# crisbodnar/text-to-image

Measured on AMD Instinct MI355X. Metric: images/sec (G+D step) at 64x64 batch=64, higher is better.
Workload: dtype f32; 1 GPU; wgancls 64x64 batch=64/GPU fp32, synthetic images + random 1024-d text embeddings, D step (+kt) then G step, Adam(b1=0,b2=0.9); global_batch=64, parallelism=dp1, launch=hipGraph replay (1 graph/iteration)

## Files before the change

### text-to-image_amd/csrc/t2i_thin.hip

```cpp
#include <hip/hip_runtime.h>
#include <stdint.h>

#include "t2i_internal.h"

namespace t2i {

template <int CI, bool DYH = false>
__global__ __launch_bounds__(256) void thin_deconv_k4s2_kernel(const void* __restrict__ dyv, const float* __restrict__ w,
                                                               const float* __restrict__ bias, float* __restrict__ dx,
                                                               int H, int W, int Co, int CH, int act, float alpha) {
  extern __shared__ __attribute__((aligned(16))) float tile[];
  const int Ho = H >> 1, Wo = W >> 1;
  const int PS = CH + 4;
  const int b = blockIdx.z;
  const int ih0 = blockIdx.y * 16, iw0 = blockIdx.x * 16;
  const int oh0 = (ih0 >> 1) - 1, ow0 = (iw0 >> 1) - 1;
  const int c4n = CH >> 2;
  float* wlds = tile + 100 * PS;
  const int wv = __builtin_amdgcn_readfirstlane(threadIdx.x >> 6);
  const int ph = wv >> 1, pw = wv & 1;
  const int lane = threadIdx.x & 63;
  const int py = lane >> 3, px = lane & 7;
  const int kh0 = (ph + 1) & 1, kw0 = (pw + 1) & 1;
  float acc[CI];
#pragma unroll
  for (int ci = 0; ci < CI; ++ci) acc[ci] = 0.f;
  for (int cbase = 0; cbase < Co; cbase += CH) {
    if (cbase) __syncthreads();
    if (CH == 64) {
      constexpr int C4N = 16, XN = (100 * C4N + 255) / 256, WN = (16 * CI * C4N + 255) / 256;
      float4 xv[XN], wv[WN];
#pragma unroll
      for (int u = 0; u < XN; ++u) {
        const int i = threadIdx.x + 256 * u;
        const int pix = i >> 4, c4 = i & 15;
        const int r = pix / 10, c = pix - r * 10;
        const int oh = oh0 + r, ow = ow0 + c;
        float4 v = make_float4(0.f, 0.f, 0.f, 0.f);
        if (i < 100 * C4N && (unsigned)oh < (unsigned)Ho && (unsigned)ow < (unsigned)Wo) {
          const size_t e = ((size_t)(b * Ho + oh) * Wo + ow) * Co + cbase + c4 * 4;
          if (DYH) {
            const uint2 q = *reinterpret_cast<const uint2*>(reinterpret_cast<const unsigned short*>(dyv) + e);
            v = make_float4(__uint_as_float(q.x << 16), __uint_as_float(q.x & 0xFFFF0000u), __uint_as_float(q.y << 16), __uint_as_float(q.y & 0xFFFF0000u));
          } else {
            v = *reinterpret_cast<const float4*>(reinterpret_cast<const float*>(dyv) + e);
          }
        }
        xv[u] = v;
      }
#pragma unroll
      for (int u = 0; u < WN; ++u) {
        const int i = threadIdx.x + 256 * u;
        const int row = i >> 4, c4 = i & 15;
        wv[u] = i < 16 * CI * C4N ? *reinterpret_cast<const float4*>(w + (size_t)row * Co + cbase + c4 * 4) : make_float4(0.f, 0.f, 0.f, 0.f);
      }
#pragma unroll
      for (int u = 0; u < XN; ++u) {
        const int i = threadIdx.x + 256 * u;
        if (i < 100 * C4N) *reinterpret_cast<float4*>(&tile[(i >> 4) * PS + (i & 15) * 4]) = xv[u];
      }
#pragma unroll
      for (int u = 0; u < WN; ++u) {
        const int i = threadIdx.x + 256 * u;
        if (i < 16 * CI * C4N) reinterpret_cast<float4*>(wlds)[i] = wv[u];
      }
    } else {
    for (int i = threadIdx.x; i < 100 * c4n; i += 256) {
      const int pix = i / c4n, c4 = i - pix * c4n;
      const int r = pix / 10, c = pix - r * 10;
      const int oh = oh0 + r, ow = ow0 + c;
      float4 v = make_float4(0.f, 0.f, 0.f, 0.f);
      if ((unsigned)oh < (unsigned)Ho && (unsigned)ow < (unsigned)Wo) {
        const size_t e = ((size_t)(b * Ho + oh) * Wo + ow) * Co + cbase + c4 * 4;
        if (DYH) {
          const uint2 u = *reinterpret_cast<const uint2*>(reinterpret_cast<const unsigned short*>(dyv) + e);
          v = make_float4(__uint_as_float(u.x << 16), __uint_as_float(u.x & 0xFFFF0000u), __uint_as_float(u.y << 16), __uint_as_float(u.y & 0xFFFF0000u));
        } else {
          v = *reinterpret_cast<const float4*>(reinterpret_cast<const float*>(dyv) + e);
        }
      }
      *reinterpret_cast<float4*>(&tile[pix * PS + c4 * 4]) = v;
    }
    for (int i = threadIdx.x; i < 16 * CI * c4n; i += 256) {
      const int row = i / c4n, c4 = i - row * c4n;
      reinterpret_cast<float4*>(wlds)[i] = *reinterpret_cast<const float4*>(w + (size_t)row * Co + cbase + c4 * 4);
    }
    }
    __syncthreads();
#pragma unroll
    for (int jh = 0; jh < 2; ++jh) {
#pragma unroll
      for (int jw = 0; jw < 2; ++jw) {
        const int r = py + 1 + ph - jh, c = px + 1 + pw - jw;
        const float* src = &tile[(r * 10 + c) * PS];
        const float* wt = wlds + (((kh0 + 2 * jh) * 4 + (kw0 + 2 * jw)) * CI) * CH;
#pragma unroll 4
        for (int c4 = 0; c4 < c4n; ++c4) {
          const float4 d = *reinterpret_cast<const float4*>(src + c4 * 4);
#pragma unroll
          for (int ci = 0; ci < CI; ++ci) {
            const float4 f = *reinterpret_cast<const float4*>(wt + ci * CH + c4 * 4);
            acc[ci] = fmaf(d.x, f.x, fmaf(d.y, f.y, fmaf(d.z, f.z, fmaf(d.w, f.w, acc[ci]))));
          }
        }
      }
    }
  }
  const int ih = ih0 + 2 * py + ph, iw = iw0 + 2 * px + pw;
  float* o = dx + ((size_t)(b * H + ih) * W + iw) * CI;
#pragma unroll
  for (int ci = 0; ci < CI; ++ci) o[ci] = apply_act(acc[ci] + (bias ? bias[ci] : 0.f), act, alpha);
}

bool thin_deconv_eligible(const t2i_conv_desc& d) {
  return d.KH == 4 && d.KW == 4 && d.SH == 2 && d.SW == 2 && d.pad_t == 1 && d.pad_l == 1 && d.Cin >= 1 && d.Cin <= 4 &&
         (d.Cout % 4) == 0 && d.Cout >= 16 && d.Cout <= 512 && (d.H % 16) == 0 && (d.W % 16) == 0 && d.Ho * 2 == d.H &&
         d.Wo * 2 == d.W;
}

hipError_t thin_deconv_launch(const t2i_conv_desc& d, const void* dy, const float* w, const float* bias, float* dx,
                              int act, float alpha, hipStream_t stream, bool dy_bf16) {
  int parts = tuning().thin_parts;
  if (parts < 1) parts = 1;
  while (parts > 1 && ((d.Cout % (4 * parts)) != 0 || d.Cout / parts < 32)) parts >>= 1;
  const int CH = d.Cout / parts;
  const size_t lds = ((size_t)100 * (CH + 4) + (size_t)16 * d.Cin * CH) * sizeof(float);
  dim3 grid(d.W / 16, d.H / 16, d.B);
#define T2I_THIN(CI)                                                                                              \
  case CI: {                                                                                                      \
    auto k = dy_bf16 ? thin_deconv_k4s2_kernel<CI, true> : thin_deconv_k4s2_kernel<CI, false>;                    \
    if (lds > 48 * 1024) {                                                                                        \
      hipError_t e = hipFuncSetAttribute(reinterpret_cast<const void*>(k), hipFuncAttributeMaxDynamicSharedMemorySize, (int)lds); \
      if (e != hipSuccess) return e;                                                                              \
    }                                                                                                             \
    hipLaunchKernelGGL(k, grid, dim3(256), lds, stream, dy, w, bias, dx, d.H, d.W, d.Cout, CH, act, alpha);       \
    break;                                                                                                        \
  }
  switch (d.Cin) {
    T2I_THIN(1) T2I_THIN(2) T2I_THIN(3) T2I_THIN(4)
    default: return hipErrorInvalidValue;
  }
#undef T2I_THIN
  return hipGetLastError();
}

template <bool BWD>
__global__ __launch_bounds__(256) void tiny_conv_kernel(const float* __restrict__ in, const float* __restrict__ w,
                                                        const float* __restrict__ bias, float* __restrict__ out,
                                                        t2i_conv_desc d, int act, float alpha) {
  const int OH = BWD ? d.H : d.Ho, OW = BWD ? d.W : d.Wo, OC = BWD ? d.Cin : d.Cout;
  const int IH = BWD ? d.Ho : d.H, IW = BWD ? d.Wo : d.W, IC = BWD ? d.Cout : d.Cin;
  const size_t npix = (size_t)d.B * OH * OW;
  for (size_t p = (size_t)blockIdx.x * blockDim.x + threadIdx.x; p < npix; p += (size_t)gridDim.x * blockDim.x) {
    const int ow = (int)(p % OW);
    const size_t t = p / OW;
    const int oh = (int)(t % OH);
    const int b = (int)(t / OH);
    float acc[4] = {0.f, 0.f, 0.f, 0.f};
    for (int kh = 0; kh < d.KH; ++kh) {
      const int ih = BWD ? oh + d.pad_t - kh : oh * d.SH - d.pad_t + kh;
      if ((unsigned)ih >= (unsigned)IH) continue;
      for (int kw = 0; kw < d.KW; ++kw) {
        const int iw = BWD ? ow + d.pad_l - kw : ow * d.SW - d.pad_l + kw;
        if ((unsigned)iw >= (unsigned)IW) continue;
        const float* src = in + ((size_t)(b * IH + ih) * IW + iw) * IC;
        const float* wt = w + (size_t)(kh * d.KW + kw) * d.Cin * d.Cout;
        for (int ic = 0; ic < IC; ++ic) {
          const float v = src[ic];
#pragma unroll
          for (int oc = 0; oc < 4; ++oc)
            if (oc < OC) acc[oc] = fmaf(v, BWD ? wt[oc * d.Cout + ic] : wt[ic * d.Cout + oc], acc[oc]);
        }
      }
    }
    float* o = out + p * OC;
#pragma unroll
    for (int oc = 0; oc < 4; ++oc)
      if (oc < OC) o[oc] = apply_act(acc[oc] + (bias ? bias[oc] : 0.f), act, alpha);
  }
}

bool tiny_conv_eligible(const t2i_conv_desc& d, bool bwd) {
  if (d.Cin > 4 || d.Cout > 4) return false;
  if (bwd && (d.SH != 1 || d.SW != 1)) return false;
  return true;
}

hipError_t tiny_conv_launch(const t2i_conv_desc& d, bool bwd, const float* in, const float* w, const float* bias,
                            float* out, int act, float alpha, hipStream_t stream) {
  const size_t npix = (size_t)d.B * (bwd ? d.H * d.W : d.Ho * d.Wo);
  size_t blocks = (npix + 255) / 256;
  if (blocks > 4096) blocks = 4096;
  if (blocks < 1) blocks = 1;
  if (bwd)
    hipLaunchKernelGGL(tiny_conv_kernel<true>, dim3((unsigned)blocks), dim3(256), 0, stream, in, w, bias, out, d, act, alpha);
  else
    hipLaunchKernelGGL(tiny_conv_kernel<false>, dim3((unsigned)blocks), dim3(256), 0, stream, in, w, bias, out, d, act, alpha);
  return hipGetLastError();
}

}

namespace t2i {

__global__ __launch_bounds__(256) void head_fwd_kernel(const float* __restrict__ x, const float* __restrict__ w,
                                                       const float* __restrict__ bias, float* __restrict__ y, int K,
                                                       int Co, int act, float alpha) {
  __shared__ float red[4][4];
  const float* row = x + (size_t)blockIdx.x * K;
  float acc[4] = {0.f, 0.f, 0.f, 0.f};
  if (Co == 1 && (K & 3) == 0 && ((reinterpret_cast<uintptr_t>(x) | reinterpret_cast<uintptr_t>(w)) & 15) == 0) {
    float4 a4 = make_float4(0.f, 0.f, 0.f, 0.f);
#pragma unroll 4
    for (int j = threadIdx.x; j < (K >> 2); j += 256) {
      const float4 v = reinterpret_cast<const float4*>(row)[j];
      const float4 q = reinterpret_cast<const float4*>(w)[j];
      a4.x = fmaf(v.x, q.x, a4.x); a4.y = fmaf(v.y, q.y, a4.y); a4.z = fmaf(v.z, q.z, a4.z); a4.w = fmaf(v.w, q.w, a4.w);
    }
    acc[0] = (a4.x + a4.y) + (a4.z + a4.w);
  } else
  for (int j = threadIdx.x; j < K; j += 256) {
    const float v = row[j];
#pragma unroll
    for (int co = 0; co < 4; ++co)
      if (co < Co) acc[co] = fmaf(v, w[(size_t)j * Co + co], acc[co]);
  }
#pragma unroll
  for (int co = 0; co < 4; ++co) {
#pragma unroll
    for (int o = 32; o > 0; o >>= 1) acc[co] += __shfl_xor(acc[co], o, 64);
    if ((threadIdx.x & 63) == 0) red[threadIdx.x >> 6][co] = acc[co];
  }
  __syncthreads();
  if (threadIdx.x < Co) {
    const int co = threadIdx.x;
    const float s = (red[0][co] + red[1][co]) + (red[2][co] + red[3][co]) + (bias ? bias[co] : 0.f);
    y[(size_t)blockIdx.x * Co + co] = apply_act(s, act, alpha);
  }
}

__global__ __launch_bounds__(256) void head_bwd_data_kernel(const float* __restrict__ dy, const float* __restrict__ w,
                                                            float* __restrict__ dx, int B, int K, int Co) {
  const size_t n = (size_t)B * K;
  for (size_t i = (size_t)blockIdx.x * blockDim.x + threadIdx.x; i < n; i += (size_t)gridDim.x * blockDim.x) {
    const size_t b = i / K;
    const int j = (int)(i - b * K);
    float s = 0.f;
    for (int co = 0; co < Co; ++co) s = fmaf(dy[b * Co + co], w[(size_t)j * Co + co], s);
    dx[i] = s;
  }
}

__global__ __launch_bounds__(256) void head_bwd_filter_kernel(const float* __restrict__ x, const float* __restrict__ dy,
                                                              float* __restrict__ dw, int B, int K, int Co, int accumulate) {
  __shared__ float red[4][64][4];
  const int tx = threadIdx.x & 63, ty = threadIdx.x >> 6;
  const int j = blockIdx.x * 64 + tx;
  float acc[4] = {0.f, 0.f, 0.f, 0.f};
  if (j < K) {
    for (int b = ty; b < B; b += 4) {
      const float v = x[(size_t)b * K + j];
#pragma unroll
      for (int co = 0; co < 4; ++co)
        if (co < Co) acc[co] = fmaf(v, dy[b * Co + co], acc[co]);
    }
  }
#pragma unroll
  for (int co = 0; co < 4; ++co) red[ty][tx][co] = acc[co];
  __syncthreads();
  if (ty == 0 && j < K) {
#pragma unroll
    for (int co = 0; co < 4; ++co)
      if (co < Co) {
        const float s = (red[0][tx][co] + red[1][tx][co]) + (red[2][tx][co] + red[3][tx][co]);
        float* o = dw + (size_t)j * Co + co;
        *o = accumulate ? *o + s : s;
      }
  }
}

bool head_conv_eligible(const t2i_conv_desc& d) {
  return d.Ho == 1 && d.Wo == 1 && d.KH == d.H && d.KW == d.W && d.pad_t == 0 && d.pad_l == 0 && d.Cout <= 4;
}

hipError_t head_fwd_launch(const t2i_conv_desc& d, const float* x, const float* w, const float* bias, float* y, int act,
                           float alpha, hipStream_t stream) {
  hipLaunchKernelGGL(head_fwd_kernel, dim3(d.B), dim3(256), 0, stream, x, w, bias, y, d.H * d.W * d.Cin, d.Cout, act, alpha);
  return hipGetLastError();
}

hipError_t head_bwd_data_launch(const t2i_conv_desc& d, const float* dy, const float* w, float* dx, hipStream_t stream) {
  const int K = d.H * d.W * d.Cin;
  size_t blocks = ((size_t)d.B * K + 255) / 256;
  if (blocks > 4096) blocks = 4096;
  hipLaunchKernelGGL(head_bwd_data_kernel, dim3((unsigned)blocks), dim3(256), 0, stream, dy, w, dx, d.B, K, d.Cout);
  return hipGetLastError();
}

hipError_t head_bwd_filter_launch(const t2i_conv_desc& d, const float* x, const float* dy, float* dw, int accumulate,
                                  hipStream_t stream) {
  const int K = d.H * d.W * d.Cin;
  hipLaunchKernelGGL(head_bwd_filter_kernel, dim3((K + 63) / 64), dim3(256), 0, stream, x, dy, dw, d.B, K, d.Cout, accumulate);
  return hipGetLastError();
}

}

namespace t2i {

typedef float f32x16_t __attribute__((ext_vector_type(16)));

template <int CI, int NB>
__global__ __launch_bounds__(256) void stem_k4s2_fwd_kernel(const float* __restrict__ x, const float* __restrict__ w,
                                                            const float* __restrict__ bias, float* __restrict__ y, int H, int W,
                                                            int act, float alpha, __bf16* __restrict__ yh) {
  constexpr int K = 16 * CI, Co = 32 * NB;
  extern __shared__ __attribute__((aligned(16))) float lds_stem[];
  const int Wo = W >> 1, Ho = H >> 1;
  constexpr int cols = 66 * CI;
  float* xs = lds_stem;
  float* ws = lds_stem + 10 * cols;
  const int b = blockIdx.z, oh0 = blockIdx.y * 4, ow0 = blockIdx.x * 32;
  constexpr int XN = (10 * cols + 255) / 256, WN = (K * Co / 4 + 255) / 256;
  float xv[XN];
  float4 wv[WN];
#pragma unroll
  for (int u = 0; u < XN; ++u) {
    const int i = threadIdx.x + 256 * u;
    const int r = i / cols, j = i - r * cols;
    const int px = j / CI, ci = j - px * CI;
    const int ih = 2 * oh0 - 1 + r, iw = 2 * ow0 - 1 + px;
    const bool ok = i < 10 * cols && (unsigned)ih < (unsigned)H && (unsigned)iw < (unsigned)W;
    xv[u] = ok ? x[((size_t)(b * H + ih) * W + iw) * CI + ci] : 0.f;
  }
#pragma unroll
  for (int u = 0; u < WN; ++u) {
    const int i = threadIdx.x + 256 * u;
    wv[u] = i < K * Co / 4 ? reinterpret_cast<const float4*>(w)[i] : make_float4(0.f, 0.f, 0.f, 0.f);
  }
#pragma unroll
  for (int u = 0; u < XN; ++u) {
    const int i = threadIdx.x + 256 * u;
    if (i < 10 * cols) xs[i] = xv[u];
  }
#pragma unroll
  for (int u = 0; u < WN; ++u) {
    const int i = threadIdx.x + 256 * u;
    if (i < K * Co / 4) reinterpret_cast<float4*>(ws)[i] = wv[u];
  }
  __syncthreads();
  const int lane = threadIdx.x & 63, wave = threadIdx.x >> 6;
  const int l31 = lane & 31, lh = lane >> 5;
  f32x16_t acc[NB];
#pragma unroll
  for (int j = 0; j < NB; ++j)
#pragma unroll
    for (int e = 0; e < 16; ++e) acc[j][e] = 0.f;
#pragma unroll
  for (int s2 = 0; s2 < K / 2; ++s2) {
    const int k = 2 * s2 + lh;
    const int tap = k / CI, ci = k - tap * CI;
    const int kh = tap >> 2, kw = tap & 3;
    const float a = xs[(2 * wave + kh) * cols + (2 * l31 + kw) * CI + ci];
#pragma unroll
    for (int j = 0; j < NB; ++j)
      acc[j] = __builtin_amdgcn_mfma_f32_32x32x2f32(a, ws[k * Co + j * 32 + l31], acc[j], 0, 0, 0);
  }
  const int oh = oh0 + wave;
  if constexpr (NB % 2 == 0) {
    constexpr int SROW = 68;
    __syncthreads();
    float* st = lds_stem + wave * (32 * SROW);
#pragma unroll
    for (int half = 0; half < NB / 2; ++half) {
#pragma unroll
      for (int jj = 0; jj < 2; ++jj)
#pragma unroll
        for (int e = 0; e < 16; ++e) st[((e & 3) + 8 * (e >> 2) + 4 * lh) * SROW + jj * 32 + l31] = acc[half * 2 + jj][e];
      __builtin_amdgcn_fence(__ATOMIC_RELEASE, "wavefront");
      __builtin_amdgcn_wave_barrier();
      __builtin_amdgcn_fence(__ATOMIC_ACQUIRE, "wavefront");
#pragma unroll
      for (int it = 0; it < 4; ++it) {
        const int idx = it * 64 + lane, row = idx >> 3, c8 = idx & 7;
        const float4 v0 = *reinterpret_cast<const float4*>(&st[row * SROW + c8 * 8]);
        const float4 v1 = *reinterpret_cast<const float4*>(&st[row * SROW + c8 * 8 + 4]);
        const int ow = ow0 + row, ch = half * 64 + c8 * 8;
        if (oh < Ho && ow < Wo) {
          float v[8] = {v0.x, v0.y, v0.z, v0.w, v1.x, v1.y, v1.z, v1.w};
          if (bias) {
            const float4 b0 = *reinterpret_cast<const float4*>(bias + ch), b1 = *reinterpret_cast<const float4*>(bias + ch + 4);
            v[0] += b0.x; v[1] += b0.y; v[2] += b0.z; v[3] += b0.w; v[4] += b1.x; v[5] += b1.y; v[6] += b1.z; v[7] += b1.w;
          } else {
#pragma unroll
            for (int k = 0; k < 8; ++k) v[k] += 0.f;
          }
#pragma unroll
          for (int k = 0; k < 8; ++k) v[k] = apply_act(v[k], act, alpha);
          const size_t o = ((size_t)(b * Ho + oh) * Wo + ow) * Co + ch;
          if (y) {
            *reinterpret_cast<float4*>(y + o) = make_float4(v[0], v[1], v[2], v[3]);
            *reinterpret_cast<float4*>(y + o + 4) = make_float4(v[4], v[5], v[6], v[7]);
          }
          if (yh) {
            typedef float f2_t __attribute__((ext_vector_type(2)));
            typedef __bf16 h2_t __attribute__((ext_vector_type(2)));
            uint4 h;
            { f2_t t = {v[0], v[1]}; h.x = __builtin_bit_cast(unsigned, __builtin_convertvector(t, h2_t)); }
            { f2_t t = {v[2], v[3]}; h.y = __builtin_bit_cast(unsigned, __builtin_convertvector(t, h2_t)); }
            { f2_t t = {v[4], v[5]}; h.z = __builtin_bit_cast(unsigned, __builtin_convertvector(t, h2_t)); }
            { f2_t t = {v[6], v[7]}; h.w = __builtin_bit_cast(unsigned, __builtin_convertvector(t, h2_t)); }
            *reinterpret_cast<uint4*>(reinterpret_cast<unsigned short*>(yh) + o) = h;
          }
        }
      }
      __builtin_amdgcn_fence(__ATOMIC_RELEASE, "wavefront");
      __builtin_amdgcn_wave_barrier();
      __builtin_amdgcn_fence(__ATOMIC_ACQUIRE, "wavefront");
    }
  } else if (oh < Ho) {
#pragma unroll
    for (int j = 0; j < NB; ++j) {
      const float bv = bias ? bias[j * 32 + l31] : 0.f;
#pragma unroll
      for (int e = 0; e < 16; ++e) {
        const int ow = ow0 + (e & 3) + 8 * (e >> 2) + 4 * lh;
        if (ow < Wo) {
          const float v = apply_act(acc[j][e] + bv, act, alpha);
          const size_t o = ((size_t)(b * Ho + oh) * Wo + ow) * Co + j * 32 + l31;
          if (y) y[o] = v;
          if (yh) yh[o] = (__bf16)v;
        }
      }
    }
  }
}

bool stem_fwd_eligible(const t2i_conv_desc& d) {
  return d.KH == 4 && d.KW == 4 && d.SH == 2 && d.SW == 2 && d.pad_t == 1 && d.pad_l == 1 && d.Cin == 3 && (d.Cout == 128 || d.Cout == 64) &&
         (d.H & 1) == 0 && (d.W & 1) == 0 && d.Ho * 2 == d.H && d.Wo * 2 == d.W;
}

hipError_t stem_fwd_launch(const t2i_conv_desc& d, const float* x, const float* w, const float* bias, float* y, int act, float alpha,
                           hipStream_t stream, void* y_h) {
  size_t lds = ((size_t)10 * 66 * 3 + (size_t)48 * d.Cout) * sizeof(float);
  if (lds < (size_t)4 * 32 * 68 * sizeof(float)) lds = (size_t)4 * 32 * 68 * sizeof(float);
  auto k = d.Cout == 128 ? stem_k4s2_fwd_kernel<3, 4> : stem_k4s2_fwd_kernel<3, 2>;
  dim3 grid((d.Wo + 31) / 32, (d.Ho + 3) / 4, d.B);
  hipLaunchKernelGGL(k, grid, dim3(256), lds, stream, x, w, bias, y, d.H, d.W, act, alpha, reinterpret_cast<__bf16*>(y_h));
  return hipGetLastError();
}

}

namespace t2i {

size_t col_reduce_ws(int64_t rows, int C);
hipError_t col_reduce_launch(const void*, const void*, const float*, int64_t, int, float*, float*, int, void*, hipStream_t, bool in_bf16 = false);

template <int CI, int CO>
__global__ __launch_bounds__(256) void tiny_bwdw_kernel(const float* __restrict__ x, const float* __restrict__ dy,
                                                        float* __restrict__ part, t2i_conv_desc d) {
  __shared__ float red[4][9 * CI * CO];
  float acc[9][CI][CO];
#pragma unroll
  for (int t = 0; t < 9; ++t)
#pragma unroll
    for (int ci = 0; ci < CI; ++ci)
#pragma unroll
      for (int co = 0; co < CO; ++co) acc[t][ci][co] = 0.f;
  const size_t npix = (size_t)d.B * d.Ho * d.Wo;
  for (size_t p = (size_t)blockIdx.x * blockDim.x + threadIdx.x; p < npix; p += (size_t)gridDim.x * blockDim.x) {
    const int ow = (int)(p % d.Wo);
    const size_t t = p / d.Wo;
    const int oh = (int)(t % d.Ho), b = (int)(t / d.Ho);
    float g[CO];
#pragma unroll
    for (int co = 0; co < CO; ++co) g[co] = dy[p * CO + co];
#pragma unroll
    for (int kh = 0; kh < 3; ++kh) {
      const int ih = oh * d.SH - d.pad_t + kh;
#pragma unroll
      for (int kw = 0; kw < 3; ++kw) {
        const int iw = ow * d.SW - d.pad_l + kw;
        if (kh < d.KH && kw < d.KW && (unsigned)ih < (unsigned)d.H && (unsigned)iw < (unsigned)d.W) {
          const float* s = x + ((size_t)(b * d.H + ih) * d.W + iw) * CI;
#pragma unroll
          for (int ci = 0; ci < CI; ++ci) {
            const float v = s[ci];
#pragma unroll
            for (int co = 0; co < CO; ++co) acc[kh * 3 + kw][ci][co] = fmaf(v, g[co], acc[kh * 3 + kw][ci][co]);
          }
        }
      }
    }
  }
#pragma unroll
  for (int t = 0; t < 9; ++t)
#pragma unroll
    for (int ci = 0; ci < CI; ++ci)
#pragma unroll
      for (int co = 0; co < CO; ++co) {
        float v = acc[t][ci][co];
#pragma unroll
        for (int o = 32; o > 0; o >>= 1) v += __shfl_xor(v, o, 64);
        if ((threadIdx.x & 63) == 0) red[threadIdx.x >> 6][(t * CI + ci) * CO + co] = v;
      }
  __syncthreads();
  if (threadIdx.x < 9 * CI * CO) {
    const int i = threadIdx.x;
    const int t = i / (CI * CO), r = i - t * (CI * CO);
    const int kh = t / 3, kw = t - kh * 3;
    if (kh < d.KH && kw < d.KW)
      part[(size_t)blockIdx.x * (d.KH * d.KW * CI * CO) + (kh * d.KW + kw) * (CI * CO) + r] =
          (red[0][i] + red[1][i]) + (red[2][i] + red[3][i]);
  }
}

typedef float stem_f32x16 __attribute__((ext_vector_type(16)));

template <bool DYH, int NB = 4>
__global__ __launch_bounds__(256) void stem_k4s2_bwdf_kernel(const float* __restrict__ x, const void* __restrict__ dy, float* __restrict__ part,
                                                             int B, int H, int W, int Ho, int Wo, int pix_per_wave, FastDiv div_wo, FastDiv div_ho) {
  extern __shared__ __attribute__((aligned(16))) float red[];
  constexpr int CO = 32 * NB;
  const int tid = threadIdx.x, lane = tid & 63, wave = tid >> 6;
  const int l31 = lane & 31, lh = lane >> 5;
  const int P = B * Ho * Wo;
  const int p_begin = (blockIdx.x * 4 + wave) * pix_per_wave;
  int p_end = p_begin + pix_per_wave;
  if (p_end > P) p_end = P;
  int a_off[2]; bool a_ok[2]; int a_kh[2], a_kw[2];
#pragma unroll
  for (int blk = 0; blk < 2; ++blk) {
    const int m = blk * 32 + l31;
    a_ok[blk] = m < 48;
    const int tap = m / 3, ci = m - tap * 3;
    a_kh[blk] = tap >> 2; a_kw[blk] = tap & 3;
    a_off[blk] = (a_kh[blk] * W + a_kw[blk]) * 3 + ci;
  }
  stem_f32x16 acc[2][NB];
#pragma unroll
  for (int i = 0; i < 2; ++i)
#pragma unroll
    for (int j = 0; j < NB; ++j)
#pragma unroll
      for (int e = 0; e < 16; ++e) acc[i][j][e] = 0.f;

  const __amdgpu_buffer_rsrc_t rx = __builtin_amdgcn_make_buffer_rsrc(const_cast<float*>(x), (short)0, (int)((size_t)B * H * W * 3 * 4), 0x00020000);
  const __amdgpu_buffer_rsrc_t ry = __builtin_amdgcn_make_buffer_rsrc(const_cast<void*>(dy), (short)0, (int)((size_t)P * CO * (DYH ? 2 : 4)), 0x00020000);
  constexpr unsigned OOB = 0xFFFFFFF0u;
  auto load = [&](int p, float (&a)[2], float (&b)[NB]) __attribute__((always_inline)) {
    const int pix = p + lh;
    const bool ok = pix < p_end;
    const int pp = ok ? pix : p_begin;
    const int t = div_wo.div(pp);
    const int ow = pp - t * Wo;
    const int img = div_ho.div(t);
    const int oh = t - img * Ho;
    const int ih0 = 2 * oh - 1, iw0 = 2 * ow - 1;
    const int xbase = ((img * H + ih0) * W + iw0) * 3;
#pragma unroll
    for (int blk = 0; blk < 2; ++blk) {
      const bool in = ok & a_ok[blk] & ((unsigned)(ih0 + a_kh[blk]) < (unsigned)H) & ((unsigned)(iw0 + a_kw[blk]) < (unsigned)W);
      a[blk] = __builtin_bit_cast(float, __builtin_amdgcn_raw_buffer_load_b32(rx, in ? (unsigned)(xbase + a_off[blk]) * 4u : OOB, 0, 0));
    }
    constexpr unsigned ES = DYH ? 2u : 4u;
    const unsigned ybase = ok ? ((unsigned)pp * (unsigned)CO + (unsigned)l31) * ES : OOB;
#pragma unroll
    for (int j = 0; j < NB; ++j) {
      if (DYH) b[j] = __uint_as_float((unsigned)(unsigned short)__builtin_amdgcn_raw_buffer_load_b16(ry, ok ? ybase + j * 32u * ES : OOB, 0, 0) << 16);
      else b[j] = __builtin_bit_cast(float, __builtin_amdgcn_raw_buffer_load_b32(ry, ok ? ybase + j * 32u * ES : OOB, 0, 0));
    }
  };

  float a0[4][2], b0[4][NB], a1[4][2], b1[4][NB];
  auto load8 = [&](int p, float (&a)[4][2], float (&b)[4][NB]) __attribute__((always_inline)) {
#pragma unroll
    for (int s = 0; s < 4; ++s) load(p + 2 * s, a[s], b[s]);
  };
  auto mma8 = [&](float (&a)[4][2], float (&b)[4][NB]) __attribute__((always_inline)) {
#pragma unroll
    for (int s = 0; s < 4; ++s)
#pragma unroll
      for (int i = 0; i < 2; ++i)
#pragma unroll
        for (int j = 0; j < NB; ++j) acc[i][j] = __builtin_amdgcn_mfma_f32_32x32x2f32(a[s][i], b[s][j], acc[i][j], 0, 0, 0);
  };
  load8(p_begin, a0, b0);
  for (int p = p_begin; p < p_end; p += 16) {
    load8(p + 8, a1, b1);
    mma8(a0, b0);
    load8(p + 16, a0, b0);
    mma8(a1, b1);
  }

  auto put = [&](float* buf) __attribute__((always_inline)) {
#pragma unroll
    for (int i = 0; i < 2; ++i)
#pragma unroll
      for (int j = 0; j < NB; ++j)
#pragma unroll
        for (int e = 0; e < 16; ++e) buf[(i * 32 + (e & 3) + 8 * (e >> 2) + 4 * lh) * CO + j * 32 + l31] = acc[i][j][e];
  };
  auto add = [&](const float* buf) __attribute__((always_inline)) {
#pragma unroll
    for (int i = 0; i < 2; ++i)
#pragma unroll
      for (int j = 0; j < NB; ++j)
#pragma unroll
        for (int e = 0; e < 16; ++e) acc[i][j][e] += buf[(i * 32 + (e & 3) + 8 * (e >> 2) + 4 * lh) * CO + j * 32 + l31];
  };
  float* buf0 = red;
  float* buf1 = red + 64 * CO;
  if (wave == 2) put(buf0);
  if (wave == 3) put(buf1);
  __syncthreads();
  if (wave == 0) add(buf0);
  if (wave == 1) add(buf1);
  __syncthreads();
  if (wave == 1) put(buf0);
  __syncthreads();
  if (wave == 0) {
    add(buf0);
    float* o = part + (size_t)blockIdx.x * 48 * CO;
#pragma unroll
    for (int i = 0; i < 2; ++i)
#pragma unroll
      for (int j = 0; j < NB; ++j)
#pragma unroll
        for (int e = 0; e < 16; ++e) {
          const int m = i * 32 + (e & 3) + 8 * (e >> 2) + 4 * lh;
          if (m < 48) o[m * CO + j * 32 + l31] = acc[i][j][e];
        }
  }
}

bool stem_bwdf_eligible(const t2i_conv_desc& d) { return stem_fwd_eligible(d); }

static int stem_bwdf_groups(const t2i_conv_desc& d, int* pix_per_wave) {
  const long P = (long)d.B * d.Ho * d.Wo;
  long ppw = (P + 1023) / 1024;
  if (ppw < 16) ppw = 16;
  ppw = (ppw + 15) & ~15L;
  *pix_per_wave = (int)ppw;
  return (int)((P + 4 * ppw - 1) / (4 * ppw));
}

size_t stem_bwdf_ws(const t2i_conv_desc& d) {
  int ppw;
  return (size_t)stem_bwdf_groups(d, &ppw) * 48 * d.Cout * sizeof(float);
}

hipError_t stem_bwdf_launch(const t2i_conv_desc& d, const float* x, const void* dy, float* dw, int accumulate, void* ws, hipStream_t stream, bool dy_bf16) {
  int ppw;
  const int G = stem_bwdf_groups(d, &ppw);
  float* part = reinterpret_cast<float*>(ws);
  const size_t lds = (size_t)2 * 64 * d.Cout * sizeof(float);
  auto k = d.Cout == 128 ? (dy_bf16 ? stem_k4s2_bwdf_kernel<true, 4> : stem_k4s2_bwdf_kernel<false, 4>)
                         : (dy_bf16 ? stem_k4s2_bwdf_kernel<true, 2> : stem_k4s2_bwdf_kernel<false, 2>);
  hipError_t e = hipFuncSetAttribute(reinterpret_cast<const void*>(k), hipFuncAttributeMaxDynamicSharedMemorySize, (int)lds);
  if (e != hipSuccess) return e;
  FastDiv dwo, dho;
  dwo.set((uint32_t)d.Wo); dho.set((uint32_t)d.Ho);
  hipLaunchKernelGGL(k, dim3(G), dim3(256), lds, stream, x, dy, part, d.B, d.H, d.W, d.Ho, d.Wo, ppw, dwo, dho);
  e = hipGetLastError();
  if (e != hipSuccess) return e;
  return splitk_reduce_launch(part, G, (size_t)48 * d.Cout, nullptr, d.Cout, T2I_ACT_NONE, 0.f, dw, accumulate, stream);
}

bool tiny_bwdw_eligible(const t2i_conv_desc& d) { return d.Cin == 3 && d.Cout == 3 && d.KH <= 3 && d.KW <= 3; }

static int tiny_bwdw_blocks(const t2i_conv_desc& d) {
  size_t npix = (size_t)d.B * d.Ho * d.Wo;
  size_t blocks = (npix + 256 * 8 - 1) / (256 * 8);
  if (blocks > 512) blocks = 512;
  if (blocks < 1) blocks = 1;
  return (int)blocks;
}

size_t tiny_bwdw_ws(const t2i_conv_desc& d) {
  const int nb = tiny_bwdw_blocks(d), C = d.KH * d.KW * 9;
  return (size_t)nb * C * sizeof(float) + col_reduce_ws(nb, C) + 256;
}

hipError_t tiny_bwdw_launch(const t2i_conv_desc& d, const float* x, const float* dy, float* dw, int accumulate, void* ws,
                            hipStream_t stream) {
  const int nb = tiny_bwdw_blocks(d), C = d.KH * d.KW * 9;
  float* part = reinterpret_cast<float*>(ws);
  char* ws2 = reinterpret_cast<char*>(ws) + (((size_t)nb * C * sizeof(float) + 255) & ~(size_t)255);
  hipLaunchKernelGGL((tiny_bwdw_kernel<3, 3>), dim3(nb), dim3(256), 0, stream, x, dy, part, d);
  return col_reduce_launch(part, nullptr, nullptr, nb, C, dw, nullptr, accumulate, ws2, stream);
}

}
```

Before: 5085 images/sec.

## Add specialized 3x3 3-channel conv kernels and vectorized head filter gradient

```diff
diff --git a/text-to-image_amd/csrc/t2i_thin.hip b/text-to-image_amd/csrc/t2i_thin.hip
--- a/text-to-image_amd/csrc/t2i_thin.hip
+++ b/text-to-image_amd/csrc/t2i_thin.hip
@@ -180,6 +180,98 @@
   }
 }
 
+template <bool V4>
+__device__ __forceinline__ void load_px6(const float* __restrict__ in, int q0, int npix, float (&v)[18]) {
+  const float* s = in + (ptrdiff_t)q0 * 3;
+  if (V4) {
+    const bool l = (unsigned)q0 < (unsigned)npix, m = (unsigned)(q0 + 1) < (unsigned)npix, r = (unsigned)(q0 + 5) < (unsigned)npix;
+    const float4 z = make_float4(0.f, 0.f, 0.f, 0.f);
+    const float4 a = m ? *reinterpret_cast<const float4*>(s + 3) : z, b = m ? *reinterpret_cast<const float4*>(s + 7) : z,
+                 c = m ? *reinterpret_cast<const float4*>(s + 11) : z;
+#pragma unroll
+    for (int e = 0; e < 3; ++e) { v[e] = l ? s[e] : 0.f; v[15 + e] = r ? s[15 + e] : 0.f; }
+    v[3] = a.x; v[4] = a.y; v[5] = a.z; v[6] = a.w; v[7] = b.x; v[8] = b.y; v[9] = b.z; v[10] = b.w;
+    v[11] = c.x; v[12] = c.y; v[13] = c.z; v[14] = c.w;
+  } else {
+#pragma unroll
+    for (int t = 0; t < 6; ++t) {
+      const bool ok = (unsigned)(q0 + t) < (unsigned)npix;
+#pragma unroll
+      for (int e = 0; e < 3; ++e) v[3 * t + e] = ok ? s[3 * t + e] : 0.f;
+    }
+  }
+}
+
+template <bool V4>
+__device__ __forceinline__ void load_nbhd4(const float* __restrict__ in, int p0, int npix, int H, int W, float (&m)[4][3][3][3]) {
+  float v[3][18];
+#pragma unroll
+  for (int r = 0; r < 3; ++r) load_px6<V4>(in, p0 - 1 + (r - 1) * W, npix, v[r]);
+  int w = p0 % W, h = (p0 / W) % H;
+#pragma unroll
+  for (int j = 0; j < 4; ++j) {
+#pragma unroll
+    for (int r = 0; r < 3; ++r)
+#pragma unroll
+      for (int c = 0; c < 3; ++c) {
+        const bool ok = (unsigned)(h + r - 1) < (unsigned)H && (unsigned)(w + c - 1) < (unsigned)W;
+#pragma unroll
+        for (int ch = 0; ch < 3; ++ch) m[j][r][c][ch] = ok ? v[r][3 * (j + c) + ch] : 0.f;
+      }
+    if (++w == W) { w = 0; if (++h == H) h = 0; }
+  }
+}
+
+template <bool BWD, bool V4>
+__global__ __launch_bounds__(256) void tiny_conv3_kernel(const float* __restrict__ in, const float* __restrict__ w,
+                                                         const float* __restrict__ bias, float* __restrict__ out, int H, int W,
+                                                         int npix, int act, float alpha) {
+  const int quads = (npix + 3) >> 2;
+  for (int q = blockIdx.x * 256 + threadIdx.x; q < quads; q += gridDim.x * 256) {
+    const int p0 = q * 4;
+    float m[4][3][3][3];
+    load_nbhd4<V4>(in, p0, npix, H, W, m);
+    float acc[4][3];
+#pragma unroll
+    for (int j = 0; j < 4; ++j)
+#pragma unroll
+      for (int oc = 0; oc < 3; ++oc) acc[j][oc] = 0.f;
+#pragma unroll
+    for (int kh = 0; kh < 3; ++kh)
+#pragma unroll
+      for (int kw = 0; kw < 3; ++kw)
+#pragma unroll
+        for (int ic = 0; ic < 3; ++ic)
+#pragma unroll
+          for (int oc = 0; oc < 3; ++oc) {
+            const float f = w[(kh * 3 + kw) * 9 + (BWD ? oc * 3 + ic : ic * 3 + oc)];
+#pragma unroll
+            for (int j = 0; j < 4; ++j) acc[j][oc] = fmaf(BWD ? m[j][2 - kh][2 - kw][ic] : m[j][kh][kw][ic], f, acc[j][oc]);
+          }
+    float o[12];
+#pragma unroll
+    for (int j = 0; j < 4; ++j)
+#pragma unroll
+      for (int oc = 0; oc < 3; ++oc) o[3 * j + oc] = apply_act(acc[j][oc] + (bias ? bias[oc] : 0.f), act, alpha);
+    float* dst = out + (size_t)p0 * 3;
+    if (V4) {
+      reinterpret_cast<float4*>(dst)[0] = make_float4(o[0], o[1], o[2], o[3]);
+      reinterpret_cast<float4*>(dst)[1] = make_float4(o[4], o[5], o[6], o[7]);
+      reinterpret_cast<float4*>(dst)[2] = make_float4(o[8], o[9], o[10], o[11]);
+    } else {
+#pragma unroll
+      for (int e = 0; e < 12; ++e)
+        if (p0 + e / 3 < npix) dst[e] = o[e];
+    }
+  }
+}
+
+static bool conv3_k3s1_same(const t2i_conv_desc& d) {
+  return d.Cin == 3 && d.Cout == 3 && d.KH == 3 && d.KW == 3 && d.SH == 1 && d.SW == 1 && d.pad_t == 1 && d.pad_l == 1 && d.Ho == d.H &&
+         d.Wo == d.W && (size_t)d.B * d.H * d.W < ((size_t)1 << 30);
+}
+static bool ptr16(const void* p) { return (reinterpret_cast<uintptr_t>(p) & 15) == 0; }
+
 bool tiny_conv_eligible(const t2i_conv_desc& d, bool bwd) {
   if (d.Cin > 4 || d.Cout > 4) return false;
   if (bwd && (d.SH != 1 || d.SW != 1)) return false;
@@ -189,6 +281,15 @@
 hipError_t tiny_conv_launch(const t2i_conv_desc& d, bool bwd, const float* in, const float* w, const float* bias,
                             float* out, int act, float alpha, hipStream_t stream) {
   const size_t npix = (size_t)d.B * (bwd ? d.H * d.W : d.Ho * d.Wo);
+  if (conv3_k3s1_same(d)) {
+    size_t qb = ((npix + 3) / 4 + 255) / 256;
+    if (qb > 4096) qb = 4096;
+    const bool v4 = (d.W & 3) == 0 && ptr16(in) && ptr16(out);
+    auto k = bwd ? (v4 ? tiny_conv3_kernel<true, true> : tiny_conv3_kernel<true, false>)
+                 : (v4 ? tiny_conv3_kernel<false, true> : tiny_conv3_kernel<false, false>);
+    hipLaunchKernelGGL(k, dim3((unsigned)qb), dim3(256), 0, stream, in, w, bias, out, d.H, d.W, (int)npix, act, alpha);
+    return hipGetLastError();
+  }
   size_t blocks = (npix + 255) / 256;
   if (blocks > 4096) blocks = 4096;
   if (blocks < 1) blocks = 1;
@@ -279,6 +380,39 @@
   }
 }
 
+__global__ __launch_bounds__(256) void head_bwd_filter_v4_kernel(const float* __restrict__ x, const float* __restrict__ dy,
+                                                                 float* __restrict__ dw, int B, int K4, int accumulate) {
+  __shared__ float4 red[16][16];
+  const int tx = threadIdx.x & 15, ty = threadIdx.x >> 4;
+  const int j4 = blockIdx.x * 16 + tx;
+  float4 acc = make_float4(0.f, 0.f, 0.f, 0.f);
+  if (j4 < K4) {
+    const float4* col = reinterpret_cast<const float4*>(x) + j4;
+#pragma unroll 8
+    for (int b = ty; b < B; b += 16) {
+      const float4 v = col[(size_t)b * K4];
+      const float g = dy[b];
+      acc.x = fmaf(v.x, g, acc.x); acc.y = fmaf(v.y, g, acc.y); acc.z = fmaf(v.z, g, acc.z); acc.w = fmaf(v.w, g, acc.w);
+    }
+  }
+  red[ty][tx] = acc;
+  __syncthreads();
+  if (ty == 0 && j4 < K4) {
+    float4 s = red[0][tx];
+#pragma unroll
+    for (int r = 1; r < 16; ++r) {
+      const float4 t = red[r][tx];
+      s.x += t.x; s.y += t.y; s.z += t.z; s.w += t.w;
+    }
+    float4* o = reinterpret_cast<float4*>(dw) + j4;
+    if (accumulate) {
+      const float4 t = *o;
+      s.x += t.x; s.y += t.y; s.z += t.z; s.w += t.w;
+    }
+    *o = s;
+  }
+}
+
 bool head_conv_eligible(const t2i_conv_desc& d) {
   return d.Ho == 1 && d.Wo == 1 && d.KH == d.H && d.KW == d.W && d.pad_t == 0 && d.pad_l == 0 && d.Cout <= 4;
 }
@@ -300,6 +434,10 @@
 hipError_t head_bwd_filter_launch(const t2i_conv_desc& d, const float* x, const float* dy, float* dw, int accumulate,
                                   hipStream_t stream) {
   const int K = d.H * d.W * d.Cin;
+  if (d.Cout == 1 && (K & 3) == 0 && ((reinterpret_cast<uintptr_t>(x) | reinterpret_cast<uintptr_t>(dw)) & 15) == 0) {
+    hipLaunchKernelGGL(head_bwd_filter_v4_kernel, dim3((K / 4 + 15) / 16), dim3(256), 0, stream, x, dy, dw, d.B, K / 4, accumulate);
+    return hipGetLastError();
+  }
   hipLaunchKernelGGL(head_bwd_filter_kernel, dim3((K + 63) / 64), dim3(256), 0, stream, x, dy, dw, d.B, K, d.Cout, accumulate);
   return hipGetLastError();
 }
@@ -517,6 +655,61 @@
   }
 }
 
+__device__ __forceinline__ float row16_sum(float v) {
+  v += __builtin_bit_cast(float, __builtin_amdgcn_update_dpp(0, __builtin_bit_cast(int, v), 0xB1, 0xF, 0xF, true));
+  v += __builtin_bit_cast(float, __builtin_amdgcn_update_dpp(0, __builtin_bit_cast(int, v), 0x4E, 0xF, 0xF, true));
+  v += __builtin_bit_cast(float, __builtin_amdgcn_update_dpp(0, __builtin_bit_cast(int, v), 0x141, 0xF, 0xF, true));
+  v += __builtin_bit_cast(float, __builtin_amdgcn_update_dpp(0, __builtin_bit_cast(int, v), 0x140, 0xF, 0xF, true));
+  return v;
+}
+
+template <bool V4>
+__global__ __launch_bounds__(256) void tiny_bwdw3_kernel(const float* __restrict__ x, const float* __restrict__ dy,
+                                                         float* __restrict__ part, int H, int W, int npix) {
+  __shared__ float red[16][81];
+  float acc[3][3][3][3];
+#pragma unroll
+  for (int i = 0; i < 81; ++i) (&acc[0][0][0][0])[i] = 0.f;
+  const int quads = (npix + 3) >> 2;
+  for (int q = blockIdx.x * 256 + threadIdx.x; q < quads; q += gridDim.x * 256) {
+    const int p0 = q * 4;
+    float g[12];
+    const float* gs = dy + (size_t)p0 * 3;
+    if (V4) {
+      const float4 a = reinterpret_cast<const float4*>(gs)[0], b = reinterpret_cast<const float4*>(gs)[1], c = reinterpret_cast<const float4*>(gs)[2];
+      g[0] = a.x; g[1] = a.y; g[2] = a.z; g[3] = a.w; g[4] = b.x; g[5] = b.y; g[6] = b.z; g[7] = b.w; g[8] = c.x; g[9] = c.y; g[10] = c.z; g[11] = c.w;
+    } else {
+#pragma unroll
+      for (int e = 0; e < 12; ++e) g[e] = p0 + e / 3 < npix ? gs[e] : 0.f;
+    }
+    float m[4][3][3][3];
+    load_nbhd4<V4>(x, p0, npix, H, W, m);
+#pragma unroll
+    for (int j = 0; j < 4; ++j)
+#pragma unroll
+      for (int kh = 0; kh < 3; ++kh)
+#pragma unroll
+        for (int kw = 0; kw < 3; ++kw)
+#pragma unroll
+          for (int ci = 0; ci < 3; ++ci)
+#pragma unroll
+            for (int co = 0; co < 3; ++co) acc[kh][kw][ci][co] = fmaf(m[j][kh][kw][ci], g[3 * j + co], acc[kh][kw][ci][co]);
+  }
+  const int row = threadIdx.x >> 4;
+#pragma unroll
+  for (int i = 0; i < 81; ++i) {
+    const float v = row16_sum((&acc[0][0][0][0])[i]);
+    if ((threadIdx.x & 15) == 0) red[row][i] = v;
+  }
+  __syncthreads();
+  if (threadIdx.x < 81) {
+    float s = red[0][threadIdx.x];
+#pragma unroll
+    for (int r = 1; r < 16; ++r) s += red[r][threadIdx.x];
+    part[(size_t)blockIdx.x * 81 + threadIdx.x] = s;
+  }
+}
+
 typedef float stem_f32x16 __attribute__((ext_vector_type(16)));
 
 template <bool DYH, int NB = 4>
@@ -674,6 +867,7 @@
 static int tiny_bwdw_blocks(const t2i_conv_desc& d) {
   size_t npix = (size_t)d.B * d.Ho * d.Wo;
   size_t blocks = (npix + 256 * 8 - 1) / (256 * 8);
+  if (conv3_k3s1_same(d)) blocks = (npix + 256 * 4 - 1) / (256 * 4);
   if (blocks > 512) blocks = 512;
   if (blocks < 1) blocks = 1;
   return (int)blocks;
@@ -689,7 +883,15 @@
   const int nb = tiny_bwdw_blocks(d), C = d.KH * d.KW * 9;
   float* part = reinterpret_cast<float*>(ws);
   char* ws2 = reinterpret_cast<char*>(ws) + (((size_t)nb * C * sizeof(float) + 255) & ~(size_t)255);
-  hipLaunchKernelGGL((tiny_bwdw_kernel<3, 3>), dim3(nb), dim3(256), 0, stream, x, dy, part, d);
+  if (conv3_k3s1_same(d)) {
+    const bool v4 = (d.W & 3) == 0 && ptr16(x) && ptr16(dy);
+    auto k = v4 ? tiny_bwdw3_kernel<true> : tiny_bwdw3_kernel<false>;
+    hipLaunchKernelGGL(k, dim3(nb), dim3(256), 0, stream, x, dy, part, d.H, d.W, (int)((size_t)d.B * d.H * d.W));
+  } else {
+    hipLaunchKernelGGL((tiny_bwdw_kernel<3, 3>), dim3(nb), dim3(256), 0, stream, x, dy, part, d);
+  }
+  hipError_t e = hipGetLastError();
+  if (e != hipSuccess) return e;
   return col_reduce_launch(part, nullptr, nullptr, nb, C, dw, nullptr, accumulate, ws2, stream);
 }
 
```

Result: no change. 5112 images/sec, median of 6 (+0.5%).
